# Dokumushikun/jittor-clip-fewshot

Measured on NVIDIA B200. Metric: images/sec (ViT-B/32 LoRA + MTA N=64 + LP++), higher is better.
Workload: dtype fp16

## Files before the change

jittor-clip-fewshot_b200/csrc/api.cu:

```cuda
#include <cmath>
#include <cstdarg>
#include <cstdio>
#include <cstdlib>
#include <cstring>
#include <map>
#include <mutex>
#include <utility>
#include <string>
#include <vector>

#include "../../include/jclip_b200.h"
#include "kernels.h"

using namespace jcb;

namespace jcb {
bool pdl_enabled() {
  static const bool on = [] { const char* e = getenv("JCB_PDL"); return e && e[0] == '1'; }();
  return on;
}
cudaError_t ensure_dynamic_smem(const void* func, size_t bytes) {
  if (bytes <= 48 * 1024) return cudaSuccess;
  int dev = 0;
  cudaError_t e = cudaGetDevice(&dev);
// ... 18 lines not shown
  cudaEvent_t copy_done[2] = {nullptr, nullptr};
  cudaEvent_t compute_done[2] = {nullptr, nullptr};
  int num_sms = 0, cc_major = 0, cc_minor = 0;
  int* dev_status = nullptr;
  int64_t chunk_views = 16384;
  int64_t host_chunk_views = 2048;
  void* ws = nullptr;
  size_t ws_bytes = 0;
  void* stage[2] = {nullptr, nullptr};
  size_t stage_bytes = 0;
  int64_t stage_seq = 0;
  bool stage_recorded[2] = {false, false};
  cudaEvent_t ticket_done[JCB_MAX_INFLIGHT] = {nullptr, nullptr, nullptr, nullptr};
  int* ticket_status = nullptr;
  int64_t next_ticket = 0, waited_ticket = 0;
  void* tta_ws = nullptr;
  size_t tta_ws_bytes = 0;
  cudaStream_t tta_last_stream = nullptr;
  cudaEvent_t tta_done = nullptr;
  void* tta_plan_host[2] = {nullptr, nullptr};
  size_t tta_plan_bytes[2] = {0, 0};
  cudaEvent_t tta_plan_copied[2] = {nullptr, nullptr};
  int tta_turn = 0;
  int cls_only_last = 0;
  bool overlapped = false;
  int64_t launches = 0;
  int ln_fold = 2;
  int operand_f16 = 1;
  int lora_applied = 0;
  char err[512] = {0};
  int graphs_on = 1;
  int64_t graph_max_views = 1024;
  uint64_t ws_gen = 0;
  std::vector<struct PipelineGraph*> graphs;
  int64_t graph_captures = 0, graph_launches = 0, graph_failures = 0;
  cudaStream_t capture_stream = nullptr;
  bool prof_on = false;
  std::vector<cudaEvent_t> prof_ev;
  std::vector<int> prof_cls;
  double prof_ms[JCB_KC_COUNT] = {0};
  int64_t prof_n[JCB_KC_COUNT] = {0};
  int64_t prof_timed[JCB_KC_COUNT] = {0};
  double prof_flops[JCB_KC_COUNT] = {0};
  double prof_bytes[JCB_KC_COUNT] = {0};
};

void graphs_clear_fwd(jcb_ctx* ctx);
// ... 210 lines not shown
         2 * align_up(n * T * 4);
}
size_t tower_ws_bytes(const jcb_vit* v, int64_t n) {
  return tower_ws_bytes_dims(v->W, v->tokens, static_cast<size_t>(v->grid) * v->grid, v->kpatch, n);
}
TowerWs tower_ws_carve_dims(size_t W, size_t T, size_t GG, size_t KP, int64_t n, Bump& b) {
  TowerWs w;
  w.big = b.take<__nv_bfloat16>(std::max(n * GG * KP, n * T * 4 * W));
  w.tokens = b.take<float>(n * T * W);
  w.ln_out = b.take<__nv_bfloat16>(n * T * W);
  w.qkv = b.take<__nv_bfloat16>(n * T * 3 * W);
  w.attn = b.take<__nv_bfloat16>(n * T * W);
  w.lora_u = b.take<__nv_bfloat16>(n * T * LORA_U_COLS);
  for (int i = 0; i < 2; ++i) w.stats[i] = b.take<float>(n * T * ((W + 255) / 256) * 2);
  for (int i = 0; i < 2; ++i) w.shift[i] = b.take<float>(n * T);
  return w;
}
TowerWs tower_ws_carve(const jcb_vit* v, int64_t n, Bump& b) {
  return tower_ws_carve_dims(v->W, v->tokens, static_cast<size_t>(v->grid) * v->grid, v->kpatch, n, b);
}

struct LnArgs {
  float* stats = nullptr;
  int slots = 0;
  const float* colsum = nullptr;
  void* out2 = nullptr;
  const float* stats_in = nullptr;
  const float* shift_in = nullptr;
  float* shift_out = nullptr;
  int64_t in_stride = 1;
  const __nv_bfloat16* A2 = nullptr;
  const __nv_bfloat16* B2 = nullptr;
  int K2 = 0;
  int64_t lda2 = 0, ldb2 = 0;
};

int run_gemm(jcb_ctx* ctx, int cls, int f16, const __nv_bfloat16* A, const __nv_bfloat16* B, int M, int N, int K,
             const float* bias, int epi, void* out, int64_t ldo, const LnArgs& ln = LnArgs()) {
  GemmArgs g;
  g.stats = ln.stats; g.stats_slots = ln.slots; g.colsum = ln.colsum; g.out2 = ln.out2; g.ldo2 = N;
  g.stats_in = ln.stats_in; g.shift_in = ln.shift_in; g.shift_out = ln.shift_out; g.stats_in_row_stride = ln.in_stride;
  g.A = A; g.B = B; g.lda = K; g.ldb = K; g.M = M; g.N = N; g.K = K; g.f16 = f16;
  g.A2 = ln.A2; g.B2 = ln.B2; g.K2 = ln.K2; g.lda2 = ln.lda2; g.ldb2 = ln.ldb2;
  g.bias = bias; g.epilogue = epi; g.out = out; g.ldo = ldo;
  const bool lnprep = epi == EPI_RESID_LNPREP_SHORT || epi == EPI_RESID_LNPREP_LONG;
  const double out_b = (epi == EPI_BIAS_BF16 || epi == EPI_BIAS_GELU_BF16 || epi == EPI_LNFOLD_BF16 || epi == EPI_LNFOLD_GELU_BF16)
                           ? 2.0 : (epi == EPI_BIAS_RESID_F32 ? 8.0 : (lnprep ? 10.0 : 4.0));
  const double bytes = 2.0 * M * (K + ln.K2) + 2.0 * N * (K + ln.K2) + out_b * M * N;
  LAUNCH_P(ctx, cls, 2.0 * M * N * (K + ln.K2), bytes, launch_gemm(g, ctx->dev_status, ctx->num_sms, ctx->stream));
  return JCB_OK;
}

int tower_blocks(TowerBase* t, int64_t n, const TowerWs& w, int causal, bool cls_row0 = false) {
  jcb_ctx* ctx = t->ctx;
  cudaStream_t s = ctx->stream;
  const int W = t->W, T = t->tokens, f16 = t->f16;
  const int M = static_cast<int>(n * T);
  const double MW = static_cast<double>(M) * W;
  int rc;
  if (ctx->ln_fold && t->layers[0].in_wf != nullptr) {
    const bool fold2 = ctx->ln_fold >= 2;
    const int slots = (W + 255) / 256;
    const bool cls_only = cls_row0 && ctx->cls_only_last && fold2 && !causal && T <= 64;
    int cur = 0;
    auto consumer = [&]() { LnArgs a; a.stats = w.stats[cur]; a.slots = slots; return a; };
    auto producer = [&](int64_t in_stride) {
      LnArgs a;
      a.stats = w.stats[cur ^ 1]; a.slots = slots; a.out2 = w.ln_out; a.shift_out = w.shift[cur ^ 1];
      a.stats_in = w.stats[cur]; a.shift_in = w.shift[cur]; a.in_stride = in_stride;
      cur ^= 1;
      return a;
    };
    for (int l = 0; l < t->L; ++l) {
      const LayerDev& L = t->layers[l];
      {
        LnArgs a = consumer();
        a.colsum = L.in_S;
        if ((rc = run_gemm(ctx, JCB_KC_GEMM_QKV, f16, w.ln_out, L.in_wf, M, 3 * W, W, L.in_c, EPI_LNFOLD_BF16, w.qkv, 3 * W, a))) return rc;
      }
      if (cls_only && l + 1 == t->L) {
        const int Mc = static_cast<int>(n);
        LAUNCH_P(ctx, JCB_KC_ATTENTION, 4.0 * n * t->heads * T * 64, static_cast<double>(n) * T * W * 4 + static_cast<double>(n) * W * 4,
                 launch_attention_cls(w.qkv, n, T, t->heads, w.attn, s, f16));
        {
          LnArgs a = producer(T);
          if ((rc = run_gemm(ctx, JCB_KC_GEMM_OUT, f16, w.attn, L.out_w, Mc, W, W, L.out_b, EPI_RESID_LNPREP_SHORT, w.tokens,
                             static_cast<int64_t>(T) * W, a))) return rc;
        }
        {
          LnArgs a = consumer();
          a.colsum = L.fc_S;
          if ((rc = run_gemm(ctx, JCB_KC_GEMM_FC1, f16, w.ln_out, L.fc_wf, Mc, 4 * W, W, L.fc_c, EPI_LNFOLD_GELU_BF16, w.big, 4 * W, a))) return rc;
        }
        if ((rc = run_gemm(ctx, JCB_KC_GEMM_FC2, f16, w.big, L.proj_w, Mc, W, 4 * W, L.proj_b, EPI_BIAS_RESID_F32, w.tokens,
                           static_cast<int64_t>(T) * W))) return rc;
        break;
      }
      LAUNCH_P(ctx, JCB_KC_ATTENTION, 4.0 * n * t->heads * T * T * 64, MW * (6 + 2),
               launch_attention(w.qkv, n, T, t->heads, w.attn, s, causal, ctx->dev_status, ctx->num_sms, f16));
      if (fold2) {
        {
          LnArgs a = producer(1);
          if ((rc = run_gemm(ctx, JCB_KC_GEMM_OUT, f16, w.attn, L.out_w, M, W, W, L.out_b, EPI_RESID_LNPREP_SHORT, w.tokens, W, a))) return rc;
        }
        LnArgs a = consumer();
        a.colsum = L.fc_S;
        if ((rc = run_gemm(ctx, JCB_KC_GEMM_FC1, f16, w.ln_out, L.fc_wf, M, 4 * W, W, L.fc_c, EPI_LNFOLD_GELU_BF16, w.big, 4 * W, a))) return rc;
      } else {
        if ((rc = run_gemm(ctx, JCB_KC_GEMM_OUT, f16, w.attn, L.out_w, M, W, W, L.out_b, EPI_BIAS_RESID_F32, w.tokens, W))) return rc;
        LAUNCH_P(ctx, JCB_KC_LAYERNORM, 0, MW * (4 + 2), launch_layernorm(w.tokens, M, W, L.ln2_g, L.ln2_b, w.ln_out, s, f16));
        if ((rc = run_gemm(ctx, JCB_KC_GEMM_FC1, f16, w.ln_out, L.fc_w, M, 4 * W, W, L.fc_b, EPI_BIAS_GELU_BF16, w.big, 4 * W))) return rc;
      }
      if (l + 1 < t->L) {
        LnArgs a = producer(1);
        if ((rc = run_gemm(ctx, JCB_KC_GEMM_FC2, f16, w.big, L.proj_w, M, W, 4 * W, L.proj_b, EPI_RESID_LNPREP_LONG, w.tokens, W, a))) return rc;
      } else if ((rc = run_gemm(ctx, JCB_KC_GEMM_FC2, f16, w.big, L.proj_w, M, W, 4 * W, L.proj_b, EPI_BIAS_RESID_F32, w.tokens, W))) {
        return rc;
      }
    }
    return JCB_OK;
  }
  auto lora_pair = [&](const __nv_bfloat16* x, const __nv_bfloat16* dn, const __nv_bfloat16* up, LnArgs* a) -> int {
// ... 8 lines not shown
    {
      LnArgs a;
      if ((rc = lora_pair(w.ln_out, L.lin_dn, L.lin_up, &a))) return rc;
      if ((rc = run_gemm(ctx, JCB_KC_GEMM_QKV, f16, w.ln_out, L.in_w, M, 3 * W, W, L.in_b, EPI_BIAS_BF16, w.qkv, 3 * W, a))) return rc;
    }
    LAUNCH_P(ctx, JCB_KC_ATTENTION, 4.0 * n * t->heads * T * T * 64, MW * (6 + 2),
             launch_attention(w.qkv, n, T, t->heads, w.attn, s, causal, ctx->dev_status, ctx->num_sms, f16));
    {
      LnArgs a;
      if ((rc = lora_pair(w.attn, L.lout_dn, L.lout_up, &a))) return rc;
      if ((rc = run_gemm(ctx, JCB_KC_GEMM_OUT, f16, w.attn, L.out_w, M, W, W, L.out_b, EPI_BIAS_RESID_F32, w.tokens, W, a))) return rc;
    }
    LAUNCH_P(ctx, JCB_KC_LAYERNORM, 0, MW * (4 + 2), launch_layernorm(w.tokens, M, W, L.ln2_g, L.ln2_b, w.ln_out, s, f16));
    if ((rc = run_gemm(ctx, JCB_KC_GEMM_FC1, f16, w.ln_out, L.fc_w, M, 4 * W, W, L.fc_b, EPI_BIAS_GELU_BF16, w.big, 4 * W))) return rc;
    if ((rc = run_gemm(ctx, JCB_KC_GEMM_FC2, f16, w.big, L.proj_w, M, W, 4 * W, L.proj_b, EPI_BIAS_RESID_F32, w.tokens, W))) return rc;
    if (l + 1 < t->L) {
      const LayerDev& Nx = t->layers[l + 1];
      LAUNCH_P(ctx, JCB_KC_LAYERNORM, 0, MW * (4 + 2), launch_layernorm(w.tokens, M, W, Nx.ln1_g, Nx.ln1_b, w.ln_out, s, f16));
    }
  }
  return JCB_OK;
}

int tower_forward(jcb_vit* v, const void* images, int dt, int64_t n, int apply_norm, const TowerWs& w) {
  jcb_ctx* ctx = v->ctx;
  cudaStream_t s = ctx->stream;
  const int W = v->cfg.width, T = v->tokens, GG = v->grid * v->grid, KP = v->kpatch;
  const int M = static_cast<int>(n * T);
  const double MW = static_cast<double>(M) * W;
  const double img_b = static_cast<double>(n) * 3 * v->cfg.resolution * v->cfg.resolution;
  const __nv_bfloat16* patches = is_patches(dt) ? static_cast<const __nv_bfloat16*>(images) : w.big;
  if (!is_patches(dt))
    LAUNCH_P(ctx, JCB_KC_IM2COL, 0, img_b * img_elem_bytes(dt) + img_b * 2,
             launch_im2col(images, dt, n, v->cfg.resolution, v->cfg.patch, apply_norm, w.big, s, v->f16));
  float* patch_out = reinterpret_cast<float*>(w.qkv);
  int rc = run_gemm(ctx, JCB_KC_GEMM_PATCH, v->f16, patches, v->conv_w, static_cast<int>(n * GG), W, KP, nullptr, EPI_F32, patch_out, W);
  if (rc) return rc;
  LAUNCH_P(ctx, JCB_KC_EMBED_LN, 0, MW * (4 + 4 + 2), launch_embed_ln(w.tokens, n, T, W, v->cls, v->pos, v->vpt, v->cfg.vpt_tokens, v->ln_pre_g, v->ln_pre_b, v->layers[0].ln1_g,
                              v->layers[0].ln1_b, w.ln_out, s, (ctx->ln_fold && v->layers[0].in_wf) ? w.stats[0] : nullptr, (W + 255) / 256,
                              patch_out, w.shift[0], v->f16));
  return tower_blocks(v, n, w, 0, true);
}

int64_t views_bound(const jcb_ctx* ctx, bool on_host) {
  return (on_host && !ctx->overlapped) ? std::min(ctx->host_chunk_views, ctx->chunk_views) : ctx->chunk_views;
}

int64_t balanced_chunk(int64_t n, int64_t bound) {
  if (n <= bound) return n;
  const int64_t passes = (n + bound - 1) / bound;
  return (n + passes - 1) / passes;
}

int check_vit(jcb_vit* v) {
  if (!v) return JCB_E_INVALID;
  if (!v->finalized) return fail(v->ctx, JCB_E_STATE, "jcb_vit_finalize has not been called");
  return JCB_OK;
}

int encode_views(jcb_vit* v, const void* images, int dt, bool on_host, int64_t n, int apply_norm, int normalize,
                 float* out_dev, size_t ws_extra) {
  jcb_ctx* ctx = v->ctx;
  if (dt < 0 || dt > JCB_IMG_PATCHES_F16) return fail(ctx, JCB_E_INVALID, "unknown image dtype %d", dt);
  if (is_patches(dt)) {
// ... 7 lines not shown
  if (!images || !out_dev) return fail(ctx, JCB_E_INVALID, "null image / output pointer");
  const int64_t chunk = balanced_chunk(n, views_bound(ctx, on_host));
  int rc = ws_reserve(ctx, ws_extra + tower_ws_bytes(v, chunk));
  if (rc) return rc;
  Bump b(static_cast<uint8_t*>(ctx->ws) + ws_extra);
  TowerWs w = tower_ws_carve(v, chunk, b);
  const size_t view_bytes = static_cast<size_t>(3) * v->cfg.resolution * v->cfg.resolution * img_elem_bytes(dt);
  if (on_host && (rc = stage_reserve(ctx, chunk * view_bytes))) return rc;
  const int64_t lead = (on_host && n > chunk && !ctx->overlapped) ? std::max<int64_t>(chunk / 4, 1) : 0;
  const int64_t body = lead ? balanced_chunk(n - lead, chunk) : chunk;
  int64_t ci = 0;
  for (int64_t off = 0; off < n; ++ci) {
    const int64_t m = std::min(ci == 0 && lead ? lead : body, n - off);
    const void* src = static_cast<const uint8_t*>(images) + off * view_bytes;
    int buf = 0;
    if (on_host) {
      buf = static_cast<int>(ctx->stage_seq++ & 1);
      if (ctx->stage_recorded[buf]) CUDA_TRY(ctx, cudaStreamWaitEvent(ctx->copy_stream, ctx->compute_done[buf], 0));
      CUDA_TRY(ctx, cudaMemcpyAsync(ctx->stage[buf], src, m * view_bytes, cudaMemcpyHostToDevice, ctx->copy_stream));
      CUDA_TRY(ctx, cudaEventRecord(ctx->copy_done[buf], ctx->copy_stream));
      CUDA_TRY(ctx, cudaStreamWaitEvent(ctx->stream, ctx->copy_done[buf], 0));
      src = ctx->stage[buf];
    }
    if ((rc = tower_forward(v, src, dt, m, apply_norm, w))) return rc;
    LAUNCH_P(ctx, JCB_KC_TAIL, 2.0 * m * v->cfg.width * v->cfg.embed_dim,
             static_cast<double>(m) * (v->cfg.width + v->cfg.embed_dim) * 4, launch_tail(w.tokens, m, v->tokens, v->cfg.width, v->ln_post_g, v->ln_post_b, v->proj,
                            v->cfg.embed_dim, normalize, out_dev + off * v->cfg.embed_dim, ctx->stream));
    if (on_host) {
      CUDA_TRY(ctx, cudaEventRecord(ctx->compute_done[buf], ctx->stream));
      ctx->stage_recorded[buf] = true;
    }
    off += m;
  }
  return JCB_OK;
}

int sync_and_check(jcb_ctx* ctx) {
  CUDA_TRY(ctx, cudaStreamSynchronize(ctx->stream));
  int st = 0;
  CUDA_TRY(ctx, cudaMemcpy(&st, ctx->dev_status, sizeof(int), cudaMemcpyDeviceToHost));
  if (st != 0) {
    int zero = 0;
    cudaMemcpy(ctx->dev_status, &zero, sizeof(int), cudaMemcpyHostToDevice);
    return fail(ctx, JCB_E_KERNEL, "device-side kernel status %d (101 producer / 102 mma / 103 epilogue pipeline timeout)", st);
  }
  return JCB_OK;
}

}

extern "C" {

int jcb_abi_version(void) { return JCB_ABI_VERSION; }

int jcb_ctx_create(int device, jcb_ctx** out) {
  if (!out) return JCB_E_INVALID;
  *out = nullptr;
  int count = 0;
  if (cudaGetDeviceCount(&count) != cudaSuccess || count == 0) return JCB_E_NO_DEVICE;
  if (device < 0 || device >= count) return JCB_E_INVALID;
  cudaDeviceProp prop;
  if (cudaGetDeviceProperties(&prop, device) != cudaSuccess) return JCB_E_CUDA;
  if (prop.major != 10) return JCB_E_NO_DEVICE;
  jcb_ctx* ctx = new jcb_ctx();
  ctx->device = device;
  ctx->num_sms = prop.multiProcessorCount;
  {
    const char* env_cls = getenv("JCB_CLS_ONLY_LAST_BLOCK");
    ctx->cls_only_last = (env_cls && env_cls[0] == '1') ? 1 : 0;
    const char* env_op = getenv("JCB_OPERANDS");
    ctx->operand_f16 = (env_op && (env_op[0] == 'b' || env_op[0] == 'B')) ? 0 : 1;
    const char* env_lm = getenv("JCB_LORA");
    ctx->lora_applied = (env_lm && (env_lm[0] == 'a' || env_lm[0] == 'A')) ? 1 : 0;
    const char* env_g = getenv("JCB_GRAPHS");
    ctx->graphs_on = (env_g && env_g[0] == '0') ? 0 : 1;
    const char* env = getenv("JCB_LN_FOLD");
    ctx->ln_fold = env ? atoi(env) : 2;
  }
  ctx->cc_major = prop.major;
  ctx->cc_minor = prop.minor;
  DeviceGuard g(device);
  bool ok = cudaStreamCreateWithFlags(&ctx->stream, cudaStreamNonBlocking) == cudaSuccess;
  ctx->own_stream = ok;
  ok = ok && cudaStreamCreateWithFlags(&ctx->copy_stream, cudaStreamNonBlocking) == cudaSuccess;
  for (int i = 0; i < 2 && ok; ++i) {
    ok = cudaEventCreateWithFlags(&ctx->copy_done[i], cudaEventDisableTiming) == cudaSuccess &&
         cudaEventCreateWithFlags(&ctx->compute_done[i], cudaEventDisableTiming) == cudaSuccess;
  }
  for (int i = 0; ok && i < JCB_MAX_INFLIGHT; ++i)
    ok = cudaEventCreateWithFlags(&ctx->ticket_done[i], cudaEventDisableTiming | cudaEventBlockingSync) == cudaSuccess;
  ok = ok && cudaHostAlloc(reinterpret_cast<void**>(&ctx->ticket_status), JCB_MAX_INFLIGHT * sizeof(int), cudaHostAllocDefault) == cudaSuccess;
  ok = ok && cudaMalloc(&ctx->dev_status, sizeof(int)) == cudaSuccess &&
// ... 585 lines not shown
  DeviceGuard g(ctx->device);
  if (n_views == 0) return JCB_OK;
  if (n_views < 0 || !out_host) return fail(ctx, JCB_E_INVALID, "bad arguments");
  const size_t out_bytes = align_up(static_cast<size_t>(n_views) * v->cfg.embed_dim * 4);
  if ((rc = ws_reserve(ctx, out_bytes + tower_ws_bytes(v, balanced_chunk(n_views, std::min(ctx->host_chunk_views, ctx->chunk_views)))))) return rc;
  float* out_dev = static_cast<float*>(ctx->ws);
  if ((rc = encode_views(v, images_host, img_dtype, true, n_views, apply_clip_norm, normalize, out_dev, out_bytes)))
    return rc;
  CUDA_TRY(ctx, cudaMemcpyAsync(out_host, out_dev, static_cast<size_t>(n_views) * v->cfg.embed_dim * 4,
                                cudaMemcpyDeviceToHost, ctx->stream));
  return sync_and_check(ctx);
}

int jcb_vit_debug_tokens(jcb_vit* v, const void* images_dev, int img_dtype, int64_t n_views, int apply_clip_norm,
                         float* tokens_out_dev) {
  int rc = check_vit(v);
  if (rc) return rc;
  jcb_ctx* ctx = v->ctx;
  DeviceGuard g(ctx->device);
  if (n_views < 1 || n_views > ctx->chunk_views) return fail(ctx, JCB_E_INVALID, "debug_tokens: 1 <= n_views <= chunk_views");
  if ((rc = ws_reserve(ctx, tower_ws_bytes(v, n_views)))) return rc;
  Bump b(ctx->ws);
  TowerWs w = tower_ws_carve(v, n_views, b);
  if ((rc = tower_forward(v, images_dev, img_dtype, n_views, apply_clip_norm, w))) return rc;
  CUDA_TRY(ctx, cudaMemcpyAsync(tokens_out_dev, w.tokens, static_cast<size_t>(n_views) * v->tokens * v->cfg.width * 4,
                                cudaMemcpyDeviceToDevice, ctx->stream));
  return JCB_OK;
}

namespace {
int tta_ws_reserve(jcb_ctx* ctx, size_t bytes) {
  if (bytes <= ctx->tta_ws_bytes) return JCB_OK;
  CUDA_TRY(ctx, cudaDeviceSynchronize());
  if (ctx->tta_ws) cudaFree(ctx->tta_ws);
  ctx->tta_ws = nullptr;
  ctx->tta_ws_bytes = 0;
  cudaError_t e = cudaMalloc(&ctx->tta_ws, bytes);
  if (e != cudaSuccess) return fail(ctx, JCB_E_NOMEM, "cudaMalloc(%zu) for the view generator failed: %s", bytes, cudaGetErrorString(e));
  ctx->tta_ws_bytes = bytes;
  return JCB_OK;
}

int tta_run(jcb_ctx* ctx, cudaStream_t stream, const uint8_t* src_dev, const jcb_src_image* images, int32_t n_images,
            const jcb_view_job* jobs, int64_t n_jobs, int32_t size, int out_mode, int patch, int apply_norm, void* out_dev) {
  if (n_jobs < 0 || n_images < 0 || size < 8 || size > 1024) return fail(ctx, JCB_E_INVALID, "jcb_tta: bad sizes");
  if (n_jobs == 0) return JCB_OK;
  if (!src_dev || !images || !jobs || !out_dev) return fail(ctx, JCB_E_INVALID, "jcb_tta: null pointer");
// ... 568 lines not shown
```

jittor-clip-fewshot_b200/csrc/attention.cu:

```cuda
#include <cstdlib>

#include "kernels.h"
#include "ptx.cuh"

namespace jcb {

namespace {

constexpr int HD = 64;
constexpr int LDS = HD + 8;

template <int HEADS_PER_CTA, int MT, int TP, bool CAUSAL, bool F16>
__global__ void __launch_bounds__(HEADS_PER_CTA * (TP / 16 / MT) * 32)
attention_kernel(const __nv_bfloat16* __restrict__ qkv, int T, int heads, __nv_bfloat16* __restrict__ out) {
  constexpr int WPH = TP / 16 / MT;
  constexpr int ATT_THREADS = HEADS_PER_CTA * WPH * 32;
  constexpr int TILE_ELEMS = TP * LDS;
  constexpr int NT = TP / 8;
  constexpr int KS = TP / 16;
  extern __shared__ __align__(16) uint8_t att_smem[];
  __nv_bfloat16* sm = reinterpret_cast<__nv_bfloat16*>(att_smem);
  const int W = heads * HD;
  const int groups = heads / HEADS_PER_CTA;
  const long long view = blockIdx.x / groups;
// ... 140 lines not shown
  __syncwarp();
#pragma unroll
  for (int mt = 0; mt < MT; ++mt) {
    const int row = r0 + mt * 16 + (lane >> 2);
#pragma unroll
    for (int dt = 0; dt < 8; ++dt) {
      const int col = dt * 8 + 2 * (lane & 3);
      *reinterpret_cast<uint32_t*>(stage + row * LDS + col) =
          pack_h2<F16>(o[mt][dt][0] * inv_sum[mt][0], o[mt][dt][1] * inv_sum[mt][0]);
      *reinterpret_cast<uint32_t*>(stage + (row + 8) * LDS + col) =
          pack_h2<F16>(o[mt][dt][2] * inv_sum[mt][1], o[mt][dt][3] * inv_sum[mt][1]);
    }
  }
  __syncthreads();
  __nv_bfloat16* obase = out + view * T * static_cast<long long>(W) + hg * HEADS_PER_CTA * HD;
  for (int i = tid; i < T * CH_PER_ROW; i += ATT_THREADS) {
    const int row = i / CH_PER_ROW, ch = i % CH_PER_ROW;
    const int hh = ch / (HD / 8), c8 = (ch % (HD / 8)) * 8;
    const uint4 v = *reinterpret_cast<const uint4*>(sm + (hh * 3 + 0) * TILE_ELEMS + row * LDS + c8);
    *reinterpret_cast<uint4*>(obase + static_cast<long long>(row) * W + ch * 8) = v;
  }
}

template <bool F16>
__global__ void __launch_bounds__(256)
attention_cls_kernel(const __nv_bfloat16* __restrict__ qkv, long long n_items, int T, int heads,
                     __nv_bfloat16* __restrict__ out) {
  const int lane = threadIdx.x & 31;
  const long long item = static_cast<long long>(blockIdx.x) * 8 + (threadIdx.x >> 5);
  if (item >= n_items) return;
  const long long seq = item / heads;
  const int h = static_cast<int>(item % heads);
  const int W = heads * HD;
  const __nv_bfloat16* base = qkv + seq * T * (3LL * W) + h * HD;
  float q[HD];
  {
    const uint4* qp = reinterpret_cast<const uint4*>(base);
#pragma unroll
    for (int c = 0; c < HD / 8; ++c) {
      const uint4 v = __ldg(qp + c);
      const uint32_t* hh = reinterpret_cast<const uint32_t*>(&v);
#pragma unroll
      for (int e = 0; e < 4; ++e) { const float2 t = unpack_h2<F16>(hh[e]); q[8 * c + 2 * e] = t.x; q[8 * c + 2 * e + 1] = t.y; }
    }
  }
  const float scale_log2 = 0.125f * 1.4426950408889634f;
  float sc[2];
#pragma unroll
  for (int r = 0; r < 2; ++r) {
    const int j = lane + 32 * r;
    float acc = 0.f;
    if (j < T) {
      const uint4* kp = reinterpret_cast<const uint4*>(base + static_cast<long long>(j) * (3 * W) + W);
#pragma unroll
      for (int c = 0; c < HD / 8; ++c) {
        const uint4 v = __ldg(kp + c);
        const uint32_t* hh = reinterpret_cast<const uint32_t*>(&v);
#pragma unroll
        for (int e = 0; e < 4; ++e) {
          const float2 t = unpack_h2<F16>(hh[e]);
          acc = fmaf(q[8 * c + 2 * e], t.x, acc);
          acc = fmaf(q[8 * c + 2 * e + 1], t.y, acc);
        }
      }
    }
    sc[r] = j < T ? acc * scale_log2 : -INFINITY;
  }
  const float mx = warp_max(fmaxf(sc[0], sc[1]));
  float pr[2];
  pr[0] = exp2f(sc[0] - mx);
  pr[1] = exp2f(sc[1] - mx);
  const float inv = 1.0f / warp_sum(pr[0] + pr[1]);
  pr[0] = from_h<F16>(to_h<F16>(pr[0]));
  pr[1] = from_h<F16>(to_h<F16>(pr[1]));
  float o0 = 0.f, o1 = 0.f;
  const __nv_bfloat16* vbase = base + 2 * W + 2 * lane;
  for (int j = 0; j < T; ++j) {
    const float pj = __shfl_sync(0xffffffffu, pr[j >> 5], j & 31);
    const float2 v = unpack_h2<F16>(*reinterpret_cast<const uint32_t*>(vbase + static_cast<long long>(j) * (3 * W)));
    o0 = fmaf(pj, v.x, o0);
    o1 = fmaf(pj, v.y, o1);
  }
  *reinterpret_cast<uint32_t*>(out + seq * W + h * HD + 2 * lane) = pack_h2<F16>(o0 * inv, o1 * inv);
}

template <int TP, bool CAUSAL, bool F16>
cudaError_t launch_attention_cfg(const __nv_bfloat16* qkv, int64_t n_views, int T, int heads, __nv_bfloat16* out,
                                 cudaStream_t stream) {
  constexpr int SMEM = 3 * TP * LDS * 2;
  constexpr int THREADS = (TP / 16) * 32;
  {
    cudaError_t e = ensure_dynamic_smem(attention_kernel<1, 1, TP, CAUSAL, F16>, SMEM);
    if (e != cudaSuccess) return e;
  }
  const long long grid = n_views * heads;
  attention_kernel<1, 1, TP, CAUSAL, F16><<<static_cast<unsigned>(grid), THREADS, SMEM, stream>>>(qkv, T, heads, out);
  return cudaGetLastError();
}

template <bool F16>
cudaError_t launch_attention_mma(const __nv_bfloat16* qkv, int64_t n_views, int T, int heads, __nv_bfloat16* out,
                                 cudaStream_t stream, int causal) {
  if (causal) return launch_attention_cfg<80, true, F16>(qkv, n_views, T, heads, out, stream);
  if (T > 64) return launch_attention_cfg<80, false, F16>(qkv, n_views, T, heads, out, stream);
  return launch_attention_cfg<64, false, F16>(qkv, n_views, T, heads, out, stream);
}

}

cudaError_t launch_attention_cls(const __nv_bfloat16* qkv, int64_t n_views, int T, int heads, __nv_bfloat16* out,
                                 cudaStream_t stream, int f16) {
  if (T < 1 || T > 64 || heads < 1) return cudaErrorInvalidValue;
  if (n_views == 0) return cudaSuccess;
  const long long items = n_views * heads;
  const unsigned grid = static_cast<unsigned>((items + 7) / 8);
  if (f16) attention_cls_kernel<true><<<grid, 256, 0, stream>>>(qkv, items, T, heads, out);
  else attention_cls_kernel<false><<<grid, 256, 0, stream>>>(qkv, items, T, heads, out);
  return cudaGetLastError();
}

cudaError_t launch_attention(const __nv_bfloat16* qkv, int64_t n_views, int T, int heads, __nv_bfloat16* out,
                             cudaStream_t stream, int causal, int* dev_status, int num_sms, int f16) {
  if (T < 1 || T > 128 || heads < 1) return cudaErrorInvalidValue;
  if (n_views == 0) return cudaSuccess;
  static int impl = -1;
  if (impl < 0) {
    const char* env = getenv("JCB_ATT_IMPL");
    impl = (env && env[0] == 'm') ? 0 : 1;
  }
  if (impl == 1 && dev_status != nullptr && num_sms > 0 && attention_tc_supported(T, heads, causal))
    return launch_attention_tc(qkv, n_views, T, heads, out, stream, dev_status, num_sms, f16, causal);
  if (T > 80) return cudaErrorInvalidValue;
  return f16 ? launch_attention_mma<true>(qkv, n_views, T, heads, out, stream, causal)
             : launch_attention_mma<false>(qkv, n_views, T, heads, out, stream, causal);
}

}
```

jittor-clip-fewshot_b200/csrc/gemm.cu:

```cuda
#include <cstdio>
#include <cstdlib>
#include <mutex>
#include <unordered_map>
#include <vector>
#include <cudaTypedefs.h>

#include "kernels.h"
#include "ptx.cuh"

namespace jcb {

namespace {

constexpr int BLOCK_M = 128;
constexpr int BLOCK_K = 64;
constexpr int UMMA_K = 16;
#ifndef JCB_GELU_WARPS
#define JCB_GELU_WARPS 4
#endif
__host__ __device__ constexpr int epi_warps_of(int epi) {
  return (epi == EPI_BIAS_GELU_BF16 || epi == EPI_LNFOLD_GELU_BF16) ? JCB_GELU_WARPS : 4;
}

#ifndef JCB_GELU_GROUP
// ... 32 lines not shown
  static constexpr int WARP_STAGING = (is_lnprep(EPI) ? lnprep_nb(EPI) + lnprep_nh(EPI) : GROUP) * 4096;
  static constexpr int STAGING_BYTES = EPI_WARPS * WARP_STAGING;
  static constexpr int SMEM_TOTAL = is_lnprep(EPI) ? 220 * 1024 : JCB_SMEM_KB * 1024;
  static constexpr int VEC_FLOATS = (is_lnfold(EPI) ? 2 : 1) * CW;
  static constexpr int BAR_BYTES = 512;
  static constexpr int B_ROWS = BN / CTAS;
  static constexpr int A_BYTES = BLOCK_M * BLOCK_K * 2;
  static constexpr int B_BYTES = B_ROWS * BLOCK_K * 2;
  static constexpr int STAGE_BYTES = A_BYTES + B_BYTES;
  static constexpr int STAGES = (SMEM_TOTAL - STAGING_BYTES) / STAGE_BYTES;
  static constexpr int TMEM_COLS = 2 * BN;
  static constexpr int SMEM_BYTES = STAGES * STAGE_BYTES + STAGING_BYTES + EPI_WARPS * VEC_FLOATS * 4 + BAR_BYTES + 1024;
};

struct GemmDev {
  int M, N, K;
  int K2;
  const float* bias;
  void* out;
  long long ldo;
  int* status;
  float* stats;
  int stats_slots;
  const float* colsum;
  const float* stats_in;
  const float* shift_in;
  float* shift_out;
  long long stats_in_stride;
  uint32_t idesc;
  int arrive_release;
  long long* trace;
};
constexpr int TRACE_TILES = 96;
#define JCB_TRACE(slot)                                                                  \
  do {                                                                                   \
    if (p.trace != nullptr && blockIdx.x == 0 && it < TRACE_TILES) p.trace[it * 8 + (slot)] = clock64(); \
  } while (0)

template <int BN, int EPI, int CTAS, bool F16>
__device__ __forceinline__ void gemm_body(const CUtensorMap& tmA, const CUtensorMap& tmB, const CUtensorMap& tmOut,
                                          const CUtensorMap& tmOut2, const CUtensorMap& tmA2, const CUtensorMap& tmB2,
                                          const GemmDev& p) {
  using Cfg = TileCfg<BN, CTAS, EPI>;
  constexpr int STAGES = Cfg::STAGES;
  constexpr int GROUP = Cfg::GROUP;
  constexpr int WARP_STAGING = Cfg::WARP_STAGING;
// ... 261 lines not shown
          if (lane == 0) {
            tma_store_2d(&tmOut, my_stage + b * 4096, n_blk * BN + c * 32, row0);
            if (c & 1) tma_store_2d(&tmOut2, my_half + ((c >> 1) % NH) * 4096, n_blk * BN + (c - 1) * 32, row0);
            bulk_commit();
          }
        }
        ok = __all_sync(0xffffffffu, ok);
        if (row0 + lane < p.M) {
          *reinterpret_cast<float2*>(p.stats + (static_cast<long long>(row0 + lane) * p.stats_slots + n_blk) * 2) =
              make_float2(rs, rq);
          if (n_blk == 0 && p.shift_out != nullptr) p.shift_out[row0 + lane] = shift;
        }
      } else {
        constexpr bool OUT_BF16 = out_is_bf16(EPI);
        constexpr bool FOLD = is_lnfold(EPI);
        constexpr bool GELU = EPI == EPI_BIAS_GELU_BF16 || EPI == EPI_LNFOLD_GELU_BF16;
        constexpr int CHUNK_COLS = OUT_BF16 ? 64 : 32;
        constexpr int NCH = CW / CHUNK_COLS;
        uint8_t* my_stage = staging + ew * WARP_STAGING;
        float ln_r = 1.f, ln_nmr = 0.f;
        if (FOLD) {
          float su = 0.f, sq = 0.f;
          if (row0 + lane < p.M) {
            const float2* st = reinterpret_cast<const float2*>(p.stats) + static_cast<long long>(row0 + lane) * p.stats_slots;
            for (int i = 0; i < p.stats_slots; ++i) { const float2 t2 = __ldg(st + i); su += t2.x; sq += t2.y; }
          }
          const float inv_k = 1.0f / static_cast<float>(p.K);
          const float mean = su * inv_k;
          const float var = fmaxf(fmaf(sq, inv_k, -mean * mean), 0.f);
          ln_r = 1.0f / sqrtf(var + 1e-5f);
          ln_nmr = -mean * ln_r;
        }
        const uint64_t r2 = f2_pack(ln_r, ln_r), nmr2 = f2_pack(ln_nmr, ln_nmr);
        const uint64_t k05 = f2_pack(0.5f, 0.5f), k851 = f2_pack(0.851f, 0.851f);
        (void)r2; (void)nmr2; (void)k05; (void)k851;
        uint32_t v[2][CHUNK_COLS];
        auto load_chunk = [&](int c, uint32_t (&dst)[CHUNK_COLS]) {
          tmem_ld_32x32b_x32(taddr + static_cast<uint32_t>(c * CHUNK_COLS), *reinterpret_cast<uint32_t(*)[32]>(&dst[0]));
          if (OUT_BF16)
            tmem_ld_32x32b_x32(taddr + static_cast<uint32_t>(c * CHUNK_COLS + 32),
                               *reinterpret_cast<uint32_t(*)[32]>(&dst[CHUNK_COLS - 32]));
        };
        load_chunk(0, v[0]);
#pragma unroll
        for (int c = 0; c < NCH; ++c) {
          uint32_t(&cur)[CHUNK_COLS] = v[c & 1];
          uint64_t bb2[CHUNK_COLS / 2];
// ... 163 lines not shown
  tmOut2 = tmOut;
  if (is_lnprep(EPI)) {
    if (!a.out2 || !a.stats || a.stats_slots < a.N / BN) return cudaErrorInvalidValue;
    if ((a.shift_in != nullptr) != (a.stats_in != nullptr) || a.stats_in == a.stats) return cudaErrorInvalidValue;
    if (!make_tmap_2d(&tmOut2, op_dt, a.out2, a.M, a.N, a.ldo2, 32, 64)) return cudaErrorInvalidValue;
  }
  if (is_lnfold(EPI) && (!a.stats || !a.colsum || a.stats_slots < 1)) return cudaErrorInvalidValue;
  CUtensorMap tmA2 = tmA, tmB2 = tmB;
  if (a.K2 > 0) {
    if (!make_tmap_2d(&tmA2, op_dt, a.A2, a.M, a.K2, a.lda2, BLOCK_M, BLOCK_K)) return cudaErrorInvalidValue;
    if (!make_tmap_2d(&tmB2, op_dt, a.B2, a.N, a.K2, a.ldb2, Cfg::B_ROWS, BLOCK_K)) return cudaErrorInvalidValue;
  }
  auto kern = CTAS == 2 ? gemm_tcgen05_2cta_kernel<BN, EPI, F16> : gemm_tcgen05_kernel<BN, EPI, F16>;
  {
    cudaError_t e = ensure_dynamic_smem(kern, Cfg::SMEM_BYTES);
    if (e != cudaSuccess) return e;
  }
  GemmDev p;
  p.M = a.M; p.N = a.N; p.K = a.K; p.K2 = a.K2;
  p.bias = a.bias; p.out = a.out; p.ldo = a.ldo; p.status = dev_status;
  p.stats = a.stats; p.stats_slots = a.stats_slots; p.colsum = a.colsum;
  p.stats_in = a.stats_in; p.shift_in = a.shift_in; p.shift_out = a.shift_out;
  p.stats_in_stride = a.stats_in_row_stride > 0 ? a.stats_in_row_stride : 1;
  p.idesc = umma_idesc_f32acc(a.f16 != 0, BLOCK_M * CTAS, BN);
  static int arrive_release = -1;
  if (arrive_release < 0) {
    const char* env = getenv("JCB_GEMM_ARRIVE_RELEASE");
    arrive_release = (env && env[0] == '1') ? 1 : 0;
  }
  p.arrive_release = arrive_release;
  static const char* trace_path = getenv("JCB_GEMM_TRACE");
  static long long* trace_dev = nullptr;
  p.trace = nullptr;
  if (trace_path) {
    if (!trace_dev) cudaMalloc(&trace_dev, TRACE_TILES * 8 * sizeof(long long));
    cudaMemsetAsync(trace_dev, 0, TRACE_TILES * 8 * sizeof(long long), stream);
    p.trace = trace_dev;
  }
  const int tile_m = BLOCK_M * CTAS;
  const int tiles = ((a.M + tile_m - 1) / tile_m) * (a.N / BN);
  const int units = num_sms / CTAS;
  const int grid = (tiles < units ? tiles : units) * CTAS;
  {
    cudaError_t e = launch_pdl(kern, dim3(grid), dim3(Cfg::NUM_THREADS), Cfg::SMEM_BYTES, stream, 1, tmA, tmB, tmOut, tmOut2,
                               tmA2, tmB2, p);
    if (e != cudaSuccess) return e;
// ... 85 lines not shown
```

jittor-clip-fewshot_b200/csrc/kernels.h:

```cpp
#pragma once
#include <cstddef>
#include <cstdint>
#include <utility>
#include <vector>
#include <cuda_bf16.h>
#include <cuda_runtime.h>

namespace jcb {

enum TmapDtype : int { TM_F32 = 0, TM_BF16 = 1, TM_F16 = 2 };

enum GemmEpilogue : int {
  EPI_BIAS_BF16 = 0,
  EPI_BIAS_GELU_BF16 = 1,
  EPI_BIAS_RESID_F32 = 2,
  EPI_F32 = 4,
  EPI_LNFOLD_BF16 = 5,
  EPI_LNFOLD_GELU_BF16 = 6,
  EPI_RESID_LNPREP_SHORT = 7,
  EPI_RESID_LNPREP_LONG = 8,
};

struct GemmArgs {
  const __nv_bfloat16* A = nullptr;
  const __nv_bfloat16* B = nullptr;
  int64_t lda = 0, ldb = 0;
  int M = 0, N = 0, K = 0;
  const __nv_bfloat16* A2 = nullptr;
  const __nv_bfloat16* B2 = nullptr;
  int64_t lda2 = 0, ldb2 = 0;
  int K2 = 0;
  const float* bias = nullptr;
  int epilogue = EPI_BIAS_BF16;
  void* out = nullptr;
  int64_t ldo = 0;
  float* stats = nullptr;
  int stats_slots = 0;
  const float* colsum = nullptr;
  void* out2 = nullptr;
  int64_t ldo2 = 0;
  int f16 = 0;
  const float* stats_in = nullptr;
  const float* shift_in = nullptr;
  float* shift_out = nullptr;
  int64_t stats_in_row_stride = 1;
};

cudaError_t launch_gemm(const GemmArgs& a, int* dev_status, int num_sms, cudaStream_t stream);
const char* gemm_init_driver_api();

enum ImageDtype : int { IMG_F32 = 0, IMG_BF16 = 1, IMG_U8 = 2 };
cudaError_t launch_im2col(const void* images, int img_dtype, int64_t n_views, int resolution, int patch,
                          int apply_norm, __nv_bfloat16* patches, cudaStream_t stream, int f16 = 0);
cudaError_t launch_embed_ln(float* tokens, int64_t n_views, int T, int W, const float* cls, const float* pos,
                            const float* vpt, int n_vpt, const float* g_pre, const float* b_pre, const float* g1,
                            const float* b1, __nv_bfloat16* y, cudaStream_t stream, float* stats = nullptr,
                            int stats_slots = 0,
                            const float* patch_out = nullptr,
                            float* shift = nullptr,
                            int f16 = 0);
cudaError_t launch_layernorm(const float* x, int64_t rows, int W, const float* g, const float* b,
                             __nv_bfloat16* y, cudaStream_t stream, int f16 = 0);
cudaError_t launch_tail(const float* tokens, int64_t n_views, int T, int W, const float* g, const float* b,
                        const float* proj, int E, int normalize, float* out, cudaStream_t stream,
                        const int* row_idx = nullptr);
cudaError_t launch_text_embed_ln(const long long* ids, int64_t n_seq, int T, int W, int vocab, const float* tok_emb,
                                 const float* pos, const float* g1, const float* b1, float* tokens, __nv_bfloat16* y,
                                 int* eot, cudaStream_t stream, float* stats = nullptr, int stats_slots = 0,
                                 float* shift = nullptr, int f16 = 0);
cudaError_t launch_attention(const __nv_bfloat16* qkv, int64_t n_views, int T, int heads, __nv_bfloat16* out,
                             cudaStream_t stream, int causal = 0, int* dev_status = nullptr, int num_sms = 0, int f16 = 0);
cudaError_t launch_attention_cls(const __nv_bfloat16* qkv, int64_t n_views, int T, int heads, __nv_bfloat16* out,
                                 cudaStream_t stream, int f16 = 0);
bool attention_tc_supported(int T, int heads, int causal);
cudaError_t launch_attention_tc(const __nv_bfloat16* qkv, int64_t n_views, int T, int heads, __nv_bfloat16* out,
                                cudaStream_t stream, int* dev_status, int num_sms, int f16 = 0, int causal = 0);
void tmap_cache_stats(uint64_t* hits, uint64_t* misses);
cudaError_t launch_cast_bf16(const float* src, __nv_bfloat16* dst, int64_t n, cudaStream_t stream, int f16 = 0);
cudaError_t launch_merge_lora_cast(const float* W, const float* A, const float* B, int rows, int cols, int r,
                                   float scaling, __nv_bfloat16* dst, cudaStream_t stream, int f16 = 0);

cudaError_t launch_merge_lora_f32(float* W, const float* A, const float* B, int rows, int cols, int r, float scaling,
                                  cudaStream_t stream);
cudaError_t launch_fold_ln(const float* W, const float* gamma, const float* beta, const float* bias, int N, int K,
                           __nv_bfloat16* Wf, float* S, float* c, cudaStream_t stream, int f16 = 0);

struct MtaParams {
  float lambda_y = 0.2f, lambda_q = 4.0f, th = 1e-6f, temperature = 1.0f;
  double k_frac = 0.3;
  int max_iter = 5;
};
constexpr int MTA_MAX_SETS = 4;
struct MtaSet {
  const float* feats;
  const float* text;
  float* out_mode;
// ... 89 lines not shown
```

Baseline: 1519.

## Enable CLS-only final transformer block by default with split Q/KV projection

The CLS-only last-block path is now on by default and can be turned off with an environment variable; the previous T<=64 restriction is removed. In the final layer, the QKV projection is split in two. K and V are computed for all tokens, while Q is computed only for the CLS row, using strided A and LN-stats access that the GEMM now supports. The regular attention kernel then runs, and only CLS rows go through out-proj, FC1 and FC2. This removes most of the final layer's GEMM work for non-CLS tokens. In exchange it adds an extra GEMM launch, runs full attention on uninitialized Q rows whose outputs are never used, and drops the dedicated CLS attention kernel.

```diff
diff --git a/jittor-clip-fewshot_b200/csrc/api.cu b/jittor-clip-fewshot_b200/csrc/api.cu
--- a/jittor-clip-fewshot_b200/csrc/api.cu
+++ b/jittor-clip-fewshot_b200/csrc/api.cu
@@ -64,7 +64,7 @@
   size_t tta_plan_bytes[2] = {0, 0};
   cudaEvent_t tta_plan_copied[2] = {nullptr, nullptr};
   int tta_turn = 0;
-  int cls_only_last = 0;
+  int cls_only_last = 1;
   bool overlapped = false;
   int64_t launches = 0;
   int ln_fold = 2;
@@ -321,6 +321,7 @@
 
 struct LnArgs {
   float* stats = nullptr;
+  int64_t stride = 1;
   int slots = 0;
   const float* colsum = nullptr;
   void* out2 = nullptr;
@@ -335,11 +336,12 @@
 };
 
 int run_gemm(jcb_ctx* ctx, int cls, int f16, const __nv_bfloat16* A, const __nv_bfloat16* B, int M, int N, int K,
-             const float* bias, int epi, void* out, int64_t ldo, const LnArgs& ln = LnArgs()) {
+             const float* bias, int epi, void* out, int64_t ldo, const LnArgs& ln = LnArgs(), int64_t lda = 0) {
   GemmArgs g;
   g.stats = ln.stats; g.stats_slots = ln.slots; g.colsum = ln.colsum; g.out2 = ln.out2; g.ldo2 = N;
+  g.stats_row_stride = ln.stride;
   g.stats_in = ln.stats_in; g.shift_in = ln.shift_in; g.shift_out = ln.shift_out; g.stats_in_row_stride = ln.in_stride;
-  g.A = A; g.B = B; g.lda = K; g.ldb = K; g.M = M; g.N = N; g.K = K; g.f16 = f16;
+  g.A = A; g.B = B; g.lda = lda ? lda : K; g.ldb = K; g.M = M; g.N = N; g.K = K; g.f16 = f16;
   g.A2 = ln.A2; g.B2 = ln.B2; g.K2 = ln.K2; g.lda2 = ln.lda2; g.ldb2 = ln.ldb2;
   g.bias = bias; g.epilogue = epi; g.out = out; g.ldo = ldo;
   const bool lnprep = epi == EPI_RESID_LNPREP_SHORT || epi == EPI_RESID_LNPREP_LONG;
@@ -360,7 +362,7 @@
   if (ctx->ln_fold && t->layers[0].in_wf != nullptr) {
     const bool fold2 = ctx->ln_fold >= 2;
     const int slots = (W + 255) / 256;
-    const bool cls_only = cls_row0 && ctx->cls_only_last && fold2 && !causal && T <= 64;
+    const bool cls_only = cls_row0 && ctx->cls_only_last && fold2 && !causal;
     int cur = 0;
     auto consumer = [&]() { LnArgs a; a.stats = w.stats[cur]; a.slots = slots; return a; };
     auto producer = [&](int64_t in_stride) {
@@ -372,31 +374,39 @@
     };
     for (int l = 0; l < t->L; ++l) {
       const LayerDev& L = t->layers[l];
-      {
+      const bool last_cls = cls_only && l + 1 == t->L;
+      if (!last_cls) {
         LnArgs a = consumer();
         a.colsum = L.in_S;
         if ((rc = run_gemm(ctx, JCB_KC_GEMM_QKV, f16, w.ln_out, L.in_wf, M, 3 * W, W, L.in_c, EPI_LNFOLD_BF16, w.qkv, 3 * W, a))) return rc;
+      } else {
+        LnArgs a = consumer();
+        a.colsum = L.in_S + W;
+        if ((rc = run_gemm(ctx, JCB_KC_GEMM_QKV, f16, w.ln_out, L.in_wf + static_cast<size_t>(W) * W, M, 2 * W, W, L.in_c + W,
+                           EPI_LNFOLD_BF16, w.qkv + W, 3 * W, a))) return rc;
+        a.colsum = L.in_S;
+        a.stride = T;
+        if ((rc = run_gemm(ctx, JCB_KC_GEMM_QKV, f16, w.ln_out, L.in_wf, static_cast<int>(n), W, W, L.in_c, EPI_LNFOLD_BF16,
+                           w.qkv, static_cast<int64_t>(T) * 3 * W, a, static_cast<int64_t>(T) * W))) return rc;
       }
-      if (cls_only && l + 1 == t->L) {
+      LAUNCH_P(ctx, JCB_KC_ATTENTION, 4.0 * n * t->heads * T * T * 64, MW * (6 + 2),
+               launch_attention(w.qkv, n, T, t->heads, w.attn, s, causal, ctx->dev_status, ctx->num_sms, f16));
+      if (last_cls) {
         const int Mc = static_cast<int>(n);
-        LAUNCH_P(ctx, JCB_KC_ATTENTION, 4.0 * n * t->heads * T * 64, static_cast<double>(n) * T * W * 4 + static_cast<double>(n) * W * 4,
-                 launch_attention_cls(w.qkv, n, T, t->heads, w.attn, s, f16));
+        const int64_t ldt = static_cast<int64_t>(T) * W;
         {
           LnArgs a = producer(T);
           if ((rc = run_gemm(ctx, JCB_KC_GEMM_OUT, f16, w.attn, L.out_w, Mc, W, W, L.out_b, EPI_RESID_LNPREP_SHORT, w.tokens,
-                             static_cast<int64_t>(T) * W, a))) return rc;
+                             ldt, a, ldt))) return rc;
         }
         {
           LnArgs a = consumer();
           a.colsum = L.fc_S;
           if ((rc = run_gemm(ctx, JCB_KC_GEMM_FC1, f16, w.ln_out, L.fc_wf, Mc, 4 * W, W, L.fc_c, EPI_LNFOLD_GELU_BF16, w.big, 4 * W, a))) return rc;
         }
-        if ((rc = run_gemm(ctx, JCB_KC_GEMM_FC2, f16, w.big, L.proj_w, Mc, W, 4 * W, L.proj_b, EPI_BIAS_RESID_F32, w.tokens,
-                           static_cast<int64_t>(T) * W))) return rc;
+        if ((rc = run_gemm(ctx, JCB_KC_GEMM_FC2, f16, w.big, L.proj_w, Mc, W, 4 * W, L.proj_b, EPI_BIAS_RESID_F32, w.tokens, ldt))) return rc;
         break;
       }
-      LAUNCH_P(ctx, JCB_KC_ATTENTION, 4.0 * n * t->heads * T * T * 64, MW * (6 + 2),
-               launch_attention(w.qkv, n, T, t->heads, w.attn, s, causal, ctx->dev_status, ctx->num_sms, f16));
       if (fold2) {
         {
           LnArgs a = producer(1);
@@ -451,7 +461,7 @@
   return JCB_OK;
 }
 
-int tower_forward(jcb_vit* v, const void* images, int dt, int64_t n, int apply_norm, const TowerWs& w) {
+int tower_forward(jcb_vit* v, const void* images, int dt, int64_t n, int apply_norm, const TowerWs& w, bool cls_row0) {
   jcb_ctx* ctx = v->ctx;
   cudaStream_t s = ctx->stream;
   const int W = v->cfg.width, T = v->tokens, GG = v->grid * v->grid, KP = v->kpatch;
@@ -468,7 +478,7 @@
   LAUNCH_P(ctx, JCB_KC_EMBED_LN, 0, MW * (4 + 4 + 2), launch_embed_ln(w.tokens, n, T, W, v->cls, v->pos, v->vpt, v->cfg.vpt_tokens, v->ln_pre_g, v->ln_pre_b, v->layers[0].ln1_g,
                               v->layers[0].ln1_b, w.ln_out, s, (ctx->ln_fold && v->layers[0].in_wf) ? w.stats[0] : nullptr, (W + 255) / 256,
                               patch_out, w.shift[0], v->f16));
-  return tower_blocks(v, n, w, 0, true);
+  return tower_blocks(v, n, w, 0, cls_row0);
 }
 
 int64_t views_bound(const jcb_ctx* ctx, bool on_host) {
@@ -522,7 +532,7 @@
       CUDA_TRY(ctx, cudaStreamWaitEvent(ctx->stream, ctx->copy_done[buf], 0));
       src = ctx->stage[buf];
     }
-    if ((rc = tower_forward(v, src, dt, m, apply_norm, w))) return rc;
+    if ((rc = tower_forward(v, src, dt, m, apply_norm, w, true))) return rc;
     LAUNCH_P(ctx, JCB_KC_TAIL, 2.0 * m * v->cfg.width * v->cfg.embed_dim,
              static_cast<double>(m) * (v->cfg.width + v->cfg.embed_dim) * 4, launch_tail(w.tokens, m, v->tokens, v->cfg.width, v->ln_post_g, v->ln_post_b, v->proj,
                             v->cfg.embed_dim, normalize, out_dev + off * v->cfg.embed_dim, ctx->stream));
@@ -567,7 +577,7 @@
   ctx->num_sms = prop.multiProcessorCount;
   {
     const char* env_cls = getenv("JCB_CLS_ONLY_LAST_BLOCK");
-    ctx->cls_only_last = (env_cls && env_cls[0] == '1') ? 1 : 0;
+    ctx->cls_only_last = (env_cls && env_cls[0] == '0') ? 0 : 1;
     const char* env_op = getenv("JCB_OPERANDS");
     ctx->operand_f16 = (env_op && (env_op[0] == 'b' || env_op[0] == 'B')) ? 0 : 1;
     const char* env_lm = getenv("JCB_LORA");
@@ -1199,7 +1209,7 @@
   if ((rc = ws_reserve(ctx, tower_ws_bytes(v, n_views)))) return rc;
   Bump b(ctx->ws);
   TowerWs w = tower_ws_carve(v, n_views, b);
-  if ((rc = tower_forward(v, images_dev, img_dtype, n_views, apply_clip_norm, w))) return rc;
+  if ((rc = tower_forward(v, images_dev, img_dtype, n_views, apply_clip_norm, w, false))) return rc;
   CUDA_TRY(ctx, cudaMemcpyAsync(tokens_out_dev, w.tokens, static_cast<size_t>(n_views) * v->tokens * v->cfg.width * 4,
                                 cudaMemcpyDeviceToDevice, ctx->stream));
   return JCB_OK;
diff --git a/jittor-clip-fewshot_b200/csrc/attention.cu b/jittor-clip-fewshot_b200/csrc/attention.cu
--- a/jittor-clip-fewshot_b200/csrc/attention.cu
+++ b/jittor-clip-fewshot_b200/csrc/attention.cu
@@ -186,68 +186,6 @@
   }
 }
 
-template <bool F16>
-__global__ void __launch_bounds__(256)
-attention_cls_kernel(const __nv_bfloat16* __restrict__ qkv, long long n_items, int T, int heads,
-                     __nv_bfloat16* __restrict__ out) {
-  const int lane = threadIdx.x & 31;
-  const long long item = static_cast<long long>(blockIdx.x) * 8 + (threadIdx.x >> 5);
-  if (item >= n_items) return;
-  const long long seq = item / heads;
-  const int h = static_cast<int>(item % heads);
-  const int W = heads * HD;
-  const __nv_bfloat16* base = qkv + seq * T * (3LL * W) + h * HD;
-  float q[HD];
-  {
-    const uint4* qp = reinterpret_cast<const uint4*>(base);
-#pragma unroll
-    for (int c = 0; c < HD / 8; ++c) {
-      const uint4 v = __ldg(qp + c);
-      const uint32_t* hh = reinterpret_cast<const uint32_t*>(&v);
-#pragma unroll
-      for (int e = 0; e < 4; ++e) { const float2 t = unpack_h2<F16>(hh[e]); q[8 * c + 2 * e] = t.x; q[8 * c + 2 * e + 1] = t.y; }
-    }
-  }
-  const float scale_log2 = 0.125f * 1.4426950408889634f;
-  float sc[2];
-#pragma unroll
-  for (int r = 0; r < 2; ++r) {
-    const int j = lane + 32 * r;
-    float acc = 0.f;
-    if (j < T) {
-      const uint4* kp = reinterpret_cast<const uint4*>(base + static_cast<long long>(j) * (3 * W) + W);
-#pragma unroll
-      for (int c = 0; c < HD / 8; ++c) {
-        const uint4 v = __ldg(kp + c);
-        const uint32_t* hh = reinterpret_cast<const uint32_t*>(&v);
-#pragma unroll
-        for (int e = 0; e < 4; ++e) {
-          const float2 t = unpack_h2<F16>(hh[e]);
-          acc = fmaf(q[8 * c + 2 * e], t.x, acc);
-          acc = fmaf(q[8 * c + 2 * e + 1], t.y, acc);
-        }
-      }
-    }
-    sc[r] = j < T ? acc * scale_log2 : -INFINITY;
-  }
-  const float mx = warp_max(fmaxf(sc[0], sc[1]));
-  float pr[2];
-  pr[0] = exp2f(sc[0] - mx);
-  pr[1] = exp2f(sc[1] - mx);
-  const float inv = 1.0f / warp_sum(pr[0] + pr[1]);
-  pr[0] = from_h<F16>(to_h<F16>(pr[0]));
-  pr[1] = from_h<F16>(to_h<F16>(pr[1]));
-  float o0 = 0.f, o1 = 0.f;
-  const __nv_bfloat16* vbase = base + 2 * W + 2 * lane;
-  for (int j = 0; j < T; ++j) {
-    const float pj = __shfl_sync(0xffffffffu, pr[j >> 5], j & 31);
-    const float2 v = unpack_h2<F16>(*reinterpret_cast<const uint32_t*>(vbase + static_cast<long long>(j) * (3 * W)));
-    o0 = fmaf(pj, v.x, o0);
-    o1 = fmaf(pj, v.y, o1);
-  }
-  *reinterpret_cast<uint32_t*>(out + seq * W + h * HD + 2 * lane) = pack_h2<F16>(o0 * inv, o1 * inv);
-}
-
 template <int TP, bool CAUSAL, bool F16>
 cudaError_t launch_attention_cfg(const __nv_bfloat16* qkv, int64_t n_views, int T, int heads, __nv_bfloat16* out,
                                  cudaStream_t stream) {
@@ -272,17 +210,6 @@
 
 }
 
-cudaError_t launch_attention_cls(const __nv_bfloat16* qkv, int64_t n_views, int T, int heads, __nv_bfloat16* out,
-                                 cudaStream_t stream, int f16) {
-  if (T < 1 || T > 64 || heads < 1) return cudaErrorInvalidValue;
-  if (n_views == 0) return cudaSuccess;
-  const long long items = n_views * heads;
-  const unsigned grid = static_cast<unsigned>((items + 7) / 8);
-  if (f16) attention_cls_kernel<true><<<grid, 256, 0, stream>>>(qkv, items, T, heads, out);
-  else attention_cls_kernel<false><<<grid, 256, 0, stream>>>(qkv, items, T, heads, out);
-  return cudaGetLastError();
-}
-
 cudaError_t launch_attention(const __nv_bfloat16* qkv, int64_t n_views, int T, int heads, __nv_bfloat16* out,
                              cudaStream_t stream, int causal, int* dev_status, int num_sms, int f16) {
   if (T < 1 || T > 128 || heads < 1) return cudaErrorInvalidValue;
diff --git a/jittor-clip-fewshot_b200/csrc/gemm.cu b/jittor-clip-fewshot_b200/csrc/gemm.cu
--- a/jittor-clip-fewshot_b200/csrc/gemm.cu
+++ b/jittor-clip-fewshot_b200/csrc/gemm.cu
@@ -78,6 +78,7 @@
   int* status;
   float* stats;
   int stats_slots;
+  long long stats_stride;
   const float* colsum;
   const float* stats_in;
   const float* shift_in;
@@ -385,7 +386,7 @@
         if (FOLD) {
           float su = 0.f, sq = 0.f;
           if (row0 + lane < p.M) {
-            const float2* st = reinterpret_cast<const float2*>(p.stats) + static_cast<long long>(row0 + lane) * p.stats_slots;
+            const float2* st = reinterpret_cast<const float2*>(p.stats) + static_cast<long long>(row0 + lane) * p.stats_stride * p.stats_slots;
             for (int i = 0; i < p.stats_slots; ++i) { const float2 t2 = __ldg(st + i); su += t2.x; sq += t2.y; }
           }
           const float inv_k = 1.0f / static_cast<float>(p.K);
@@ -595,6 +596,7 @@
   p.stats = a.stats; p.stats_slots = a.stats_slots; p.colsum = a.colsum;
   p.stats_in = a.stats_in; p.shift_in = a.shift_in; p.shift_out = a.shift_out;
   p.stats_in_stride = a.stats_in_row_stride > 0 ? a.stats_in_row_stride : 1;
+  p.stats_stride = a.stats_row_stride > 0 ? a.stats_row_stride : 1;
   p.idesc = umma_idesc_f32acc(a.f16 != 0, BLOCK_M * CTAS, BN);
   static int arrive_release = -1;
   if (arrive_release < 0) {
diff --git a/jittor-clip-fewshot_b200/csrc/kernels.h b/jittor-clip-fewshot_b200/csrc/kernels.h
--- a/jittor-clip-fewshot_b200/csrc/kernels.h
+++ b/jittor-clip-fewshot_b200/csrc/kernels.h
@@ -44,6 +44,7 @@
   const float* shift_in = nullptr;
   float* shift_out = nullptr;
   int64_t stats_in_row_stride = 1;
+  int64_t stats_row_stride = 1;
 };
 
 cudaError_t launch_gemm(const GemmArgs& a, int* dev_status, int num_sms, cudaStream_t stream);
@@ -70,8 +71,6 @@
                                  float* shift = nullptr, int f16 = 0);
 cudaError_t launch_attention(const __nv_bfloat16* qkv, int64_t n_views, int T, int heads, __nv_bfloat16* out,
                              cudaStream_t stream, int causal = 0, int* dev_status = nullptr, int num_sms = 0, int f16 = 0);
-cudaError_t launch_attention_cls(const __nv_bfloat16* qkv, int64_t n_views, int T, int heads, __nv_bfloat16* out,
-                                 cudaStream_t stream, int f16 = 0);
 bool attention_tc_supported(int T, int heads, int causal);
 cudaError_t launch_attention_tc(const __nv_bfloat16* qkv, int64_t n_views, int T, int heads, __nv_bfloat16* out,
                                 cudaStream_t stream, int* dev_status, int num_sms, int f16 = 0, int causal = 0);
```

Measured after the change: 1611 (median of 6 runs). 6.1% higher.
